# slowli/elastic-elgamal

Measured on AMD Instinct MI355X. Metric: EncryptedChoice ballot verifications/sec, higher is better.
Workload: dtype u32; 1 GPU; 1000000 single-choice 5-option EncryptedChoice ballots per GPU per step, resident in HBM (BASELINE.json configs[1]); verify + homomorphic tally + tally all-gather; ballots_per_gpu=1000000, total_ballots=1000000, options=5, ballot_bytes=736, seed=20260612, tampered=0, parallelism=single

## Files before the change

### elastic_elgamal_amd/csrc/eg_hip.hip

```cpp
#include <hip/hip_runtime.h>

#include <algorithm>
#include <atomic>
#include <chrono>
#include <cstdio>
#include <cstdlib>
#include <cstring>
#include <functional>
#include <memory>
#include <mutex>
#include <string>
#include <thread>
#include <condition_variable>
#include <deque>
#include <list>
#include <unordered_map>
#include <vector>

#include "../../include/eg_hip.h"
#include "host_plan.hpp"
#include "wire_json.hpp"
#include "kernels.cuh"
#include "pippenger.cuh"

// ... 146 lines not shown
  return EG_OK;
}

static void comb_table_free(uint4* tab) { if (tab) (void)hipFree(tab - COMB_HEADER_QUADS); }
static int comb_table_build(const u32* d_base_words, int bits, hipStream_t s, uint4** out, bool soft_nomem = false) {
  *out = nullptr;
  if (bits < 8 || bits > 26) return fail(EG_ERR_BAD_ARG, "comb width out of range");
  const int windows = comb_windows(bits), entries = comb_entries(bits);
  const size_t lanes = (size_t)windows * (entries / COMB_RUN);
  uint4* base = nullptr;
  u32 *d_bases = nullptr, *scratch = nullptr;
  hipError_t he = hipMalloc((void**)&base, ((size_t)windows * entries * 8 + COMB_HEADER_QUADS) * sizeof(uint4));
  if (he == hipSuccess) he = hipMalloc((void**)&d_bases, (size_t)windows * PT_WORDS * sizeof(u32));
  if (he == hipSuccess) he = hipMalloc((void**)&scratch, (size_t)COMB_RUN * EG_NL * lanes * sizeof(u32));
  if (he != hipSuccess) {
    if (base) (void)hipFree(base);
    if (d_bases) (void)hipFree(d_bases);
    if (scratch) (void)hipFree(scratch);
    if (he == hipErrorOutOfMemory && soft_nomem) { (void)hipGetLastError(); return EG_ERR_NOMEM; }
    HIPCHK(he);
  }
  hipLaunchKernelGGL(k_comb_window_bases, dim3(1), dim3(64), 0, s, d_base_words, bits, d_bases);
  hipLaunchKernelGGL(k_build_fixed_table, dim3((unsigned)((lanes + NT - 1) / NT)), dim3(NT), 0, s, d_bases, bits, base + COMB_HEADER_QUADS, scratch);
  const hipError_t se = hipStreamSynchronize(s);
  (void)hipFree(d_bases); (void)hipFree(scratch);
  if (se != hipSuccess) { (void)hipFree(base); HIPCHK(se); }
  *out = base + COMB_HEADER_QUADS;
  return EG_OK;
}

using eghost::StageDev; using eghost::LevelDev;
using eghost::FAM_TABLE1; using eghost::FAM_TABLEN; using eghost::FAM_DIRECT1; using eghost::FAM_GENERIC; using eghost::FAM_ENCODE; using eghost::N_FAM;
using eghost::EG_MULTI_GROUP; using eghost::job_family;

struct Engine {
  eg_ctx* ctx = nullptr;
  eghost::Plan plan;
  int n_options = 0;
  egplan::WireItem *d_pt_items = nullptr, *d_sc_items = nullptr;
  egplan::DeriveClass* d_dclasses = nullptr;
  egplan::DeriveTerm* d_dterms = nullptr;
  egplan::JobClass* d_jobs = nullptr;
  egplan::VarTerm* d_vterms = nullptr;
  egplan::HashInst* d_insts = nullptr;
  egplan::HashOp* d_ops = nullptr;
  egplan::StatusRule* d_rules = nullptr;
  u32* d_tally_slots = nullptr;
  unsigned short* d_base_slots = nullptr;
  egplan::SumBase* d_sum_bases = nullptr;
  unsigned short* d_sum_members = nullptr;
  egplan::SumBase* d_acc_sums = nullptr;
  unsigned short* d_acc_members = nullptr;
  int n_sums = 0;
  unsigned short* d_defer_slots = nullptr;
  int max_defer = 0;
  unsigned char* d_blob = nullptr;
  uint4 *d_tabK = nullptr, *d_cpts = nullptr;
  uint4* d_tabK_big = nullptr;
  bool use_big = false;
  size_t items_seen = 0;
  u32* d_prefixes = nullptr;
  u32* d_key_words = nullptr;
  std::vector<StageDev> stages;
  std::vector<LevelDev> levels;
  int prefix_inst_first = 0, prefix_inst_count = 0;
  struct WorkSet {
    uint4 *pts = nullptr, *cmp = nullptr, *chal = nullptr;
    u32 *states = nullptr, *flags = nullptr, *bad_item = nullptr;
    uint4 *btab = nullptr, *dpt = nullptr, *sacc = nullptr;
    u32* encw = nullptr;
    u32* partial = nullptr;
    u32* tally = nullptr;
    hipStream_t stream = nullptr;
    hipEvent_t done = nullptr;
  } set[2];
  int n_sets = 2;
  Knobs knobs;
  uint8_t key_bytes[32] = {0};
  int teeth = 6;
  hipEvent_t fork = nullptr;
  u32 cap = 0, max_cap = 0;
// ... 13 lines not shown
  bool reserved = false;
  hipEvent_t last_done = nullptr, saved_ev = nullptr;
  bool last_used = false;
  hipStream_t copy_stream = nullptr;
  unsigned char* d_wire = nullptr;
  u32* d_status = nullptr;
  size_t staging_ballots = 0;
  u32* gen_ws = nullptr;
  size_t gen_ws_bytes = 0;
  u32* d_gen_desc = nullptr;
};

static int grid_for(size_t lanes, int cap_blocks);
static int gen_workspace(Engine* e, size_t n, unsigned words, int* blocks_out) {
  const size_t budget = (size_t)2 << 30;
  int blocks = grid_for(n, e->ctx->cus * 4);
  const size_t per_block = (size_t)NT * words * sizeof(u32);
  if ((size_t)blocks * per_block > budget) blocks = (int)std::max<size_t>(1, budget / per_block);
  const size_t need = (size_t)blocks * per_block;
  if (need > e->gen_ws_bytes) {
    HIPCHK(hipDeviceSynchronize());
    if (e->gen_ws) (void)hipFree(e->gen_ws);
    e->gen_ws = nullptr; e->gen_ws_bytes = 0;
    HIPCHK(hipMalloc((void**)&e->gen_ws, need));
    e->gen_ws_bytes = need;
  }
  *blocks_out = blocks;
  return EG_OK;
}

static void engine_free(Engine* e) {
  if (!e) return;
  void* ptrs[] = {e->d_pt_items, e->d_sc_items, e->d_dclasses, e->d_dterms, e->d_jobs, e->d_vterms, e->d_insts, e->d_ops,
                  e->d_rules, e->d_tally_slots, e->d_base_slots, e->d_sum_bases, e->d_sum_members, e->d_acc_sums, e->d_acc_members, e->d_defer_slots, e->d_blob, e->d_cpts, e->d_prefixes, e->d_key_words,
                  e->tally_saved, e->tally_saved2, e->tally_saved3, e->d_tally_enc, e->d_wire, e->d_status, e->gen_ws, e->d_gen_desc};
  for (void* p : ptrs) if (p) (void)hipFree(p);
  for (auto& w : e->set) {
    void* sp[] = {w.pts, w.cmp, w.chal, w.states, w.flags, w.bad_item, w.btab, w.dpt, w.sacc, w.encw, w.partial, w.tally};
    for (void* p : sp) if (p) (void)hipFree(p);
    if (w.stream) (void)hipStreamDestroy(w.stream);
    if (w.done) (void)hipEventDestroy(w.done);
  }
  if (e->fork) (void)hipEventDestroy(e->fork);
  if (e->last_done) (void)hipEventDestroy(e->last_done);
  if (e->saved_ev) (void)hipEventDestroy(e->saved_ev);
  comb_table_free(e->d_tabK); comb_table_free(e->d_tabK_big);
  if (e->copy_stream) (void)hipStreamDestroy(e->copy_stream);
  if (e->json_ring) (void)hipHostFree(e->json_ring);
  if (e->json_status_ring) (void)hipHostFree(e->json_status_ring);
  for (hipStream_t st : e->json_ctl) if (st) (void)hipStreamDestroy(st);
  delete e;
}

static EngineBufs make_bufs(const Engine* e, int set, const void* d_ballots, u32 n, void* d_status) {
  const Engine::WorkSet& w = e->set[set];
  EngineBufs B;
  B.wire = reinterpret_cast<const u32*>(d_ballots);
  B.stride_words = (u32)(e->plan.stride / 4);
  B.n = n;
  B.cap = e->cap;
  B.pts = w.pts; B.cmp = w.cmp; B.chal = w.chal; B.states = w.states; B.flags = w.flags; B.bad_item = w.bad_item;
  B.status = reinterpret_cast<u32*>(d_status);
  B.tabG = e->use_big ? e->ctx->tabG_big : e->ctx->tabG; B.tabK = e->use_big ? e->d_tabK_big : e->d_tabK; B.cpts = e->d_cpts; B.prefixes = e->d_prefixes; B.blob = e->d_blob;
  B.ws = e->ctx->ws + (size_t)set * (e->ctx->msm_blocks / e->n_sets) * WS_QUADS * NT;
  B.btab = w.btab;
  B.sacc = w.sacc;
  B.dpt = w.dpt;
// ... 40 lines not shown
                     (void**)&w.btab, (void**)&w.dpt, (void**)&w.encw, (void**)&w.sacc};
    for (size_t i = 0; i < sizeof(sizes) / sizeof(sizes[0]); ++i) {
      const hipError_t he = hipMalloc(bufs[i], sizes[i]);
      if (he == hipErrorOutOfMemory) {
        (void)hipGetLastError();
        engine_release_sets(e);
        return fail(EG_ERR_NOMEM, "device memory exhausted while reserving the chunk workspace");
      }
      HIPCHK(he);
    }
  }
  e->cap = (u32)cap;
  return EG_OK;
}

static unsigned blocks_of(size_t n) { return (unsigned)std::max<size_t>(1, (n + NT - 1) / NT); }
static int grid_for(size_t lanes, int cap_blocks) {
  size_t blocks = (lanes + NT - 1) / NT;
  if (blocks < 1) blocks = 1;
  if ((size_t)cap_blocks < blocks) blocks = (size_t)cap_blocks;
  return (int)blocks;
}

static int engine_create(eg_ctx* ctx, eghost::Plan&& plan, const uint8_t pk[32], int n_options, Engine** out) {
  std::unique_ptr<Engine, void (*)(Engine*)> e(new Engine(), engine_free);
  e->ctx = ctx;
  e->plan = std::move(plan);
  e->n_options = n_options;
  eghost::Plan& P = e->plan;
  hipStream_t s = ctx->stream;
  HIPCHK(hipSetDevice(ctx->device));
  if (P.pk_off >= 0) memcpy(P.blob.data() + P.pk_off, pk, 32);

  const eghost::FlatPlan F = eghost::flatten_plan(P);
  {
    const std::string why = eghost::check_flat_plan(P, F);
    if (!why.empty()) return fail(EG_ERR_BAD_ARG, "internal: inconsistent verification plan: " + why);
  }
  e->stages = F.stages;
  e->levels = F.levels;
  e->max_defer = F.max_defer;
  e->prefix_inst_first = F.prefix_inst_first;
  e->prefix_inst_count = F.prefix_inst_count;
  const std::vector<egplan::JobClass>& jobs = F.jobs;
  const std::vector<egplan::HashInst>& insts = F.insts;
  const std::vector<egplan::HashOp>& ops = F.ops;
  const std::vector<uint16_t>& defer_slots = F.defer_slots;
  const std::vector<egplan::DeriveClass>& dclasses = F.dclasses;
  int rc;
  if ((rc = upload(&e->d_pt_items, P.pt_items, s))) return rc;
  if ((rc = upload(&e->d_sc_items, P.sc_items, s))) return rc;
  if ((rc = upload(&e->d_dclasses, dclasses, s))) return rc;
  if ((rc = upload(&e->d_dterms, P.dterms, s))) return rc;
  if ((rc = upload(&e->d_jobs, jobs, s))) return rc;
  if ((rc = upload(&e->d_vterms, P.vterms, s))) return rc;
  if ((rc = upload(&e->d_insts, insts, s))) return rc;
  if ((rc = upload(&e->d_ops, ops, s))) return rc;
  if ((rc = upload(&e->d_rules, P.rules, s))) return rc;
  if ((rc = upload(&e->d_tally_slots, P.tally_slots, s))) return rc;
  if ((rc = upload(&e->d_base_slots, F.build_slots, s))) return rc;
  if ((rc = upload(&e->d_sum_bases, F.sums, s))) return rc;
  if ((rc = upload(&e->d_sum_members, F.sum_members, s))) return rc;
  if ((rc = upload(&e->d_acc_sums, F.acc_sums, s))) return rc;
  if ((rc = upload(&e->d_acc_members, F.acc_members, s))) return rc;
  e->n_sums = (int)F.sums.size();
  if ((rc = upload(&e->d_defer_slots, defer_slots, s))) return rc;
  if ((rc = upload(&e->d_blob, P.blob, s))) return rc;

  u32* d_pk = nullptr;
  u32* d_flags = nullptr;
  HIPCHK(hipMalloc((void**)&d_pk, 32));
  HIPCHK(hipMalloc((void**)&d_flags, 8));
  HIPCHK(hipMalloc((void**)&e->d_key_words, 2 * PT_WORDS * sizeof(u32)));
  HIPCHK(hipMemcpyAsync(d_pk, pk, 32, hipMemcpyHostToDevice, s));
  hipLaunchKernelGGL(k_setup_points, dim3(1), dim3(64), 0, s, d_pk, e->d_key_words, d_flags);
  u32 hflags[2] = {0, 0};
  HIPCHK(hipMemcpyAsync(hflags, d_flags, 8, hipMemcpyDeviceToHost, s));
  HIPCHK(hipStreamSynchronize(s));
  (void)hipFree(d_pk); (void)hipFree(d_flags);
  if (!hflags[0]) return fail(EG_ERR_BAD_PUBLIC_KEY, "public key is not a valid ristretto255 encoding");
  if (hflags[1]) return fail(EG_ERR_BAD_PUBLIC_KEY, "public key is the identity");
  if ((rc = comb_table_build(e->d_key_words + PT_WORDS, EG_COMB_BITS, s, &e->d_tabK))) return rc;

  {
    u64* d_m = nullptr;
    std::vector<uint64_t> mults = P.const_mults;
    if (mults.empty()) mults.push_back(0);
    HIPCHK(hipMalloc((void**)&d_m, mults.size() * 8));
    HIPCHK(hipMemcpyAsync(d_m, mults.data(), mults.size() * 8, hipMemcpyHostToDevice, s));
    HIPCHK(hipMalloc((void**)&e->d_cpts, mults.size() * PT_QUADS * sizeof(uint4)));
    hipLaunchKernelGGL(k_const_points, dim3((unsigned)((mults.size() + NT - 1) / NT)), dim3(NT), 0, s, d_m, (int)mults.size(),
                       ctx->tabG, e->d_cpts);
    HIPCHK(hipStreamSynchronize(s));
// ... 133 lines not shown
    for (int k = 0; k < 2; ++k) {
      HIPCHK(hipStreamWaitEvent(e->set[k].stream, e->fork, 0));
      TRY_(ws_acquire(ctx, 1u << k, e->set[k].stream));
    }
  } else if (n) {
    TRY_(ws_acquire(ctx, 3u, s));
    whole_ws = true;
  }
  const bool inject_failure = two && EG_FAULT_POINT(after_fork);
  const int msm_blocks = ctx->msm_blocks / (two ? 2 : 1);
  size_t chunk = 0;
  for (size_t off = 0; off < n; off += even, ++chunk) {
    const int set = two ? (int)(chunk & 1) : 0;
    hipStream_t cs = two ? e->set[set].stream : s;
    const Engine::WorkSet& w = e->set[set];
    const u32 cn = (u32)std::min<size_t>(even, n - off);
    EngineBufs B = make_bufs(e, set, reinterpret_cast<const unsigned char*>(d_ballots) + off * P.stride, cn,
                             reinterpret_cast<u32*>(d_status) + off);
    if (!two) B.ws = ctx->ws;
    const int wide = ctx->cus * 32;
    HIPCHK(hipMemsetAsync(w.bad_item, 0xff, (size_t)cn * sizeof(u32), cs));
    hipLaunchKernelGGL(k_decode_points, dim3(grid_for((size_t)P.pt_items.size() * cn, wide)), dim3(NT), 0, cs, B, e->d_pt_items,
                       (int)P.pt_items.size());
    hipLaunchKernelGGL(k_check_scalars, dim3(grid_for((size_t)P.sc_items.size() * cn, wide)), dim3(NT), 0, cs, B, e->d_sc_items,
                       (int)P.sc_items.size());
    for (auto& lv : e->levels)
      if (lv.count)
        hipLaunchKernelGGL(k_derive_points, dim3(grid_for((size_t)lv.count * cn, wide)), dim3(NT), 0, cs, B, e->d_dclasses,
                           e->d_dterms, lv.first, lv.count);
    for (auto& st : e->stages) {
      if (st.build_count) {
        size_t pi = 0;
        if ((rc = prof_begin(ctx, cs, PROF_TABLES, &pi))) return rc;
        EG_WITH_TEETH(e->teeth, hipLaunchKernelGGL(k_base_tables<T>, dim3(grid_for((size_t)st.build_count * cn, msm_blocks)), dim3(NT), 0, cs, B,
                                                   e->d_base_slots + st.build_first, st.build_count));
        if ((rc = prof_end(ctx, cs, pi))) return rc;
      }
      if (st.sums_direct)
        EG_WITH_TEETH(e->teeth, hipLaunchKernelGGL(k_sum_tables<T>, dim3(grid_for((size_t)e->n_sums * cn, msm_blocks)), dim3(NT), 0, cs, B,
                                                   e->d_sum_bases, e->d_sum_members, e->n_sums));
      if (st.acc_count)
        EG_WITH_TEETH(e->teeth, hipLaunchKernelGGL(k_sum_accumulate<T>, dim3(grid_for((size_t)st.acc_count * T * cn, msm_blocks)), dim3(NT), 0, cs, B,
                                                   e->d_acc_sums + st.acc_first, e->d_acc_members, st.acc_count));
      if (st.sum_finish)
        EG_WITH_TEETH(e->teeth, hipLaunchKernelGGL(k_sum_finish<T>, dim3(grid_for((size_t)e->n_sums * cn, msm_blocks)), dim3(NT), 0, cs, B,
                                                   e->d_sum_bases, e->n_sums));
      if (st.fam_count[FAM_TABLE1]) {
        size_t pi = 0;
        if ((rc = prof_begin(ctx, cs, PROF_MSM, &pi))) return rc;
        EG_WITH_TEETH(e->teeth, hipLaunchKernelGGL((k_eq_table<false, T>), dim3(grid_for((size_t)st.fam_count[FAM_TABLE1] * cn, msm_blocks)), dim3(NT), 0, cs,
                                                   B, e->d_jobs, e->d_vterms, st.fam_first[FAM_TABLE1], st.fam_count[FAM_TABLE1], 1));
        if ((rc = prof_end(ctx, cs, pi))) return rc;
      }
      if (st.fam_count[FAM_TABLEN]) {
        const int group = std::min(st.max_terms, EG_MULTI_GROUP);
        EG_WITH_TEETH(e->teeth, hipLaunchKernelGGL((k_eq_table<true, T>), dim3(grid_for((size_t)st.fam_count[FAM_TABLEN] * cn, msm_blocks)), dim3(NT),
                                                   (size_t)group * 9 * NT * sizeof(u32), cs, B, e->d_jobs, e->d_vterms, st.fam_first[FAM_TABLEN],
                                                   st.fam_count[FAM_TABLEN], group));
      }
      if (st.fam_count[FAM_DIRECT1])
        hipLaunchKernelGGL(k_eq_direct, dim3(grid_for((size_t)st.fam_count[FAM_DIRECT1] * cn, msm_blocks)), dim3(NT), 0, cs, B,
                           e->d_jobs, e->d_vterms, st.fam_first[FAM_DIRECT1], st.fam_count[FAM_DIRECT1]);
      if (st.fam_count[FAM_GENERIC])
        EG_WITH_TEETH(e->teeth, hipLaunchKernelGGL(k_eq_generic<T>, dim3(grid_for((size_t)st.fam_count[FAM_GENERIC] * cn, msm_blocks)), dim3(NT), 0, cs, B,
                           e->d_jobs, e->d_vterms, st.fam_first[FAM_GENERIC], st.fam_count[FAM_GENERIC]));
      if (st.fam_count[FAM_ENCODE])
        hipLaunchKernelGGL(k_encode_plain, dim3(grid_for((size_t)st.fam_count[FAM_ENCODE] * cn, wide)), dim3(NT), 0, cs, B, e->d_jobs,
                           st.fam_first[FAM_ENCODE], st.fam_count[FAM_ENCODE]);
// ... 1169 lines not shown
    case 6: P = eghost::build_sumsq_plan(n_options, "test", &item); break;
    default: return fail(EG_ERR_BAD_ARG, "unknown plan kind");
  }
  size_t jobs = 0, insts = 0, var_terms = P.vterms.size(), table_terms = 0, derived = 0;
  size_t combs = 0, deferred = 0, plain_encodes = 0, inversion_groups = 0, derive_terms = P.dterms.size();
  size_t jobs_table1 = 0, chains = 0, chain_extra_terms = 0, loose_table_terms = 0, direct_terms = 0;
  std::string per_stage;
  for (auto& st : P.stages) {
    jobs += st.jobs.size(); insts += st.insts.size();
    per_stage += (per_stage.empty() ? "" : ",") + std::to_string(st.jobs.size());
    for (auto& j : st.jobs) {
      combs += (j.g.kind != egplan::SRC_NONE) + (j.k.kind != egplan::SRC_NONE);
      if (j.defer) ++deferred; else ++plain_encodes;
      switch (job_family(j, P.vterms)) {
        case FAM_TABLE1: ++jobs_table1; break;
        case FAM_TABLEN:
          for (int t0 = 0; t0 < (int)j.term_count; t0 += EG_MULTI_GROUP) {
            ++chains;
            chain_extra_terms += std::min<int>(EG_MULTI_GROUP, j.term_count - t0) - 1;
          }
          break;
        case FAM_DIRECT1: ++direct_terms; break;
        case FAM_GENERIC:
          for (unsigned t = 0; t < j.term_count; ++t)
            if (P.vterms[j.term_first + t].base == 0xffff) ++direct_terms; else ++loose_table_terms;
          break;
        default: break;
      }
    }
    inversion_groups += (st.deferred.size() + 31) / 32;
  }
  for (auto& t : P.vterms) table_terms += t.base != 0xffff;
  for (auto& l : P.derive_levels) derived += l.size();
  char tmp[2048];
  snprintf(tmp, sizeof tmp,
           "{\"stride\": %zu, \"wire_points\": %zu, \"wire_scalars\": %zu, \"derived_points\": %zu, \"derive_terms\": %zu, \"bases\": %zu, "
           "\"stages\": %zu, \"jobs\": %zu, \"jobs_per_stage\": [%s], \"var_terms\": %zu, \"table_terms\": %zu, "
           "\"combs\": %zu, \"deferred\": %zu, \"plain_encodes\": %zu, \"inversion_groups\": %zu, "
           "\"single_table_jobs\": %zu, \"chains\": %zu, \"chain_extra_terms\": %zu, \"loose_table_terms\": %zu, \"direct_terms\": %zu, "
           "\"sum_tables\": %zu, \"sum_table_members\": %zu, "
           "\"hash_programs\": %zu, \"prefixes\": %d, \"flags\": %d, \"rules\": %zu, \"tally_slots\": %zu, "
           "\"pt_slots\": %d, \"cmp_slots\": %d, \"chal_slots\": %d, \"state_slots\": %d, \"tables\": %zu, \"teeth\": %d, "
           "\"ring_group\": %d, \"table_groups\": %zu}",
           P.stride, P.pt_items.size(), P.sc_items.size(), derived, derive_terms, P.base_slots.size(), P.stages.size(), jobs, per_stage.c_str(),
           var_terms, table_terms, combs, deferred, plain_encodes, inversion_groups, jobs_table1, chains, chain_extra_terms,
           loose_table_terms, direct_terms, P.sum_bases.size(), P.sum_members.size(), insts, P.n_prefixes, P.n_flag_slots, P.rules.size(),
           P.tally_slots.size(), P.n_pt_slots, P.n_cmp_slots, P.n_chal_slots, P.n_state_slots, (size_t)P.n_tables(), eghost::plan_teeth(P),
           P.ring_group, P.group_stage.size());
  if (strlen(tmp) + 1 > cap) return fail(EG_ERR_BAD_ARG, "buffer too small");
  memcpy(buf, tmp, strlen(tmp) + 1);
  return EG_OK;
}

static int pack_json_common(const char* json, size_t json_len, int threads, size_t max_objects, size_t* n_objects,
                            std::vector<std::pair<size_t, size_t>>& spans) {
  if (!json_len) { if (n_objects) *n_objects = 0; return EG_OK; }
  if (!egwire::split_objects_parallel(json, json_len, threads, spans))
    return fail(EG_ERR_BAD_ARG, "the text is neither a JSON array of objects nor a sequence of JSON objects");
  if (n_objects) *n_objects = spans.size();
  if (spans.size() > max_objects) return fail(EG_ERR_BAD_ARG, "more objects in the text than max_objects (*n_objects says how many)");
  return EG_OK;
}
int eg_choice_pack_json(int n_options, int single, const char* json, size_t json_len, int threads, size_t max_objects,
                        uint8_t* packed, uint32_t* status, size_t* n_objects) {
  if (n_options < 1 || n_options > 4000 || (json_len && !json) || (max_objects && (!packed || !status)))
    return fail(EG_ERR_BAD_ARG, "bad argument");
  std::vector<std::pair<size_t, size_t>> spans;
  TRY(pack_json_common(json, json_len, threads, max_objects, n_objects, spans));
  const size_t stride = eghost::choice_ballot_size(n_options, single != 0);
  egwire::pack_parallel(json, spans, stride, threads, packed, status,
                        [&](egwire::Cursor& c, uint8_t* dst) { return egwire::pack_choice(c, n_options, single != 0, dst); });
  return EG_OK;
}
int eg_qv_pack_json(int n_options, uint64_t credits, const char* json, size_t json_len, int threads, size_t max_objects,
                    uint8_t* packed, uint32_t* status, size_t* n_objects) {
  if (n_options < 1 || n_options > 256 || credits < 1 || credits > 100000 || (json_len && !json) || (max_objects && (!packed || !status)))
    return fail(EG_ERR_BAD_ARG, "bad argument");
  std::vector<std::pair<size_t, size_t>> spans;
  TRY(pack_json_common(json, json_len, threads, max_objects, n_objects, spans));
  const eghost::QvShape sh = eghost::qv_shape(n_options, credits);
  const egwire::RangeShape vote{sh.vote_range.rings.size(), (size_t)sh.vote_range.rings_size()};
// ... 850 lines not shown
```

### elastic_elgamal_amd/csrc/host_plan.hpp

```cpp
#pragma once
#include <algorithm>
#include <cmath>
#include <cstdint>
#include <cstring>
#include <map>
#include <string>
#include <vector>
#include "plan.h"

namespace eghost {

using namespace egplan;

struct RingSpec { uint64_t size, step; };
struct RangeDecomposition {
  std::vector<RingSpec> rings;
  std::string to_string() const {
    std::string s;
    for (size_t i = 0; i < rings.size(); ++i) {
      if (rings[i].step > 1) s += std::to_string(rings[i].step) + " * ";
      s += "0.." + std::to_string(rings[i].size);
      if (i + 1 < rings.size()) s += " + ";
    }
    return s;
// ... 578 lines not shown
                               {OP_SAVE_PREFIX, 0, pre, 0}});
  const ScalarSrc c = wire_src(2, true), s = wire_src(3);
  const uint16_t xg = P.job(0, {}, s, c);
  const uint16_t xk = P.job(0, {P.term(dh, c), P.term(R, s)}, no_src(), no_src());
  const uint16_t flag = P.new_flag();
  P.stage(0).insts.push_back({{OP_LOAD_PREFIX, 0, pre, 0},
                              {OP_APPEND_WIRE, P.ref("K"), 0, 1},
                              {OP_APPEND_BLOB, P.ref("[r]G"), P.pk_ref(), 0},
                              {OP_APPEND_WIRE, P.ref("[r]K"), 1, 1},
                              {OP_APPEND_CMP, P.ref("[x]G"), xg, 0xffff},
                              {OP_APPEND_CMP, P.ref("[x]K"), xk, 0xffff},
                              {OP_CHALLENGE_CHECK, P.ref("c"), 2, flag}});
  P.rules.push_back({flag, 4});
  return P;
}

inline int plan_teeth(const Plan& P) {
  if (P.base_slots.empty()) return 6;
  return P.table_uses <= 2 * P.base_slots.size() + P.base_slots.size() / 2 ? 5 : 6;
}

enum { FAM_TABLE1 = 0, FAM_TABLEN = 1, FAM_DIRECT1 = 2, FAM_GENERIC = 3, FAM_ENCODE = 4, N_FAM = 5 };
constexpr int EG_MULTI_GROUP = 8;
inline int job_family(const JobClass& j, const std::vector<VarTerm>& vterms) {
  if (!j.defer) return FAM_ENCODE;
  if (j.term_count == 0) return FAM_GENERIC;
  for (unsigned t = 0; t < j.term_count; ++t)
    if (vterms[j.term_first + t].base == 0xffff) return j.term_count == 1 ? FAM_DIRECT1 : FAM_GENERIC;
  return j.term_count == 1 ? FAM_TABLE1 : FAM_TABLEN;
}
struct StageDev {
  int fam_first[N_FAM], fam_count[N_FAM], max_terms, inst_first, inst_count, defer_first, defer_count;
  int build_first, build_count, sums_direct, acc_first, acc_count, sum_finish;
};
struct LevelDev { int first, count; };
struct FlatPlan {
  std::vector<JobClass> jobs;
  std::vector<HashInst> insts;
  std::vector<HashOp> ops;
  std::vector<uint16_t> defer_slots;
  std::vector<DeriveClass> dclasses;
  std::vector<StageDev> stages;
  std::vector<LevelDev> levels;
  std::vector<uint16_t> build_slots;
  std::vector<SumBase> sums;
  std::vector<uint16_t> sum_members;
  std::vector<SumBase> acc_sums;
  std::vector<uint16_t> acc_members;
  int max_defer = 0, prefix_inst_first = 0, prefix_inst_count = 0;
};
inline FlatPlan flatten_plan(const Plan& P) {
  FlatPlan F;
  const size_t n_stages = std::max(P.stages.size(), (size_t)(P.sum_bases.empty() ? 0 : P.sum_stage + 1));
  std::vector<StageDev> tab(n_stages);
  for (auto& t : tab) t.build_first = t.build_count = t.sums_direct = t.acc_first = t.acc_count = t.sum_finish = 0;
  auto base_of = [&](uint16_t slot) -> int { auto it = P.base_index_of.find(slot); return it == P.base_index_of.end() ? -1 : (int)it->second; };
  for (size_t g = 0; g < P.group_stage.size(); ++g) {
    std::vector<uint16_t> slots(P.group_size((int)g));
    for (size_t i = 0; i < P.base_slots.size(); ++i)
      if (P.base_group[i] == g) slots[P.base_local[i]] = P.base_slots[i];
    if (slots.empty() || (size_t)P.group_stage[g] >= n_stages) continue;
    StageDev& t = tab[P.group_stage[g]];
    t.build_first = (int)F.build_slots.size(); t.build_count = (int)slots.size();
    F.build_slots.insert(F.build_slots.end(), slots.begin(), slots.end());
  }
  for (const SumBase& sb : P.sum_bases) {
    SumBase r = sb;
    r.first = (uint16_t)F.sum_members.size();
    for (unsigned t = 0; t < sb.count; ++t) {
      const int b = base_of(P.sum_members[sb.first + t]);
      F.sum_members.push_back(b < 0 ? (uint16_t)0xffff : P.base_local[b]);
    }
    F.sums.push_back(r);
  }
  if (!P.sum_bases.empty()) {
    if (!P.grouped()) tab[0].sums_direct = 1;
    else {
      std::vector<char> seen(P.sum_bases.size(), 0);
      for (size_t g = 0; g < P.group_stage.size(); ++g) {
        if ((size_t)P.group_stage[g] >= n_stages) continue;
        StageDev& t = tab[P.group_stage[g]];
        t.acc_first = (int)F.acc_sums.size();
        for (size_t k = 0; k < P.sum_bases.size(); ++k) {
          SumBase r;
          r.first = (uint16_t)F.acc_members.size(); r.count = 0; r.out_base = (uint16_t)k; r.pad = 0;
          for (unsigned m = 0; m < P.sum_bases[k].count; ++m) {
            const int b = base_of(P.sum_members[P.sum_bases[k].first + m]);
            if (b >= 0 && P.base_group[b] == g) { F.acc_members.push_back(P.base_local[b]); ++r.count; }
          }
          if (!r.count) continue;
          r.pad = seen[k] ? 0 : 1;
          seen[k] = 1;
          F.acc_sums.push_back(r);
        }
        t.acc_count = (int)F.acc_sums.size() - t.acc_first;
      }
      tab[P.sum_stage].sum_finish = 1;
    }
  }
  for (size_t si = 0; si < n_stages; ++si) {
    static const Stage empty_stage;
    const Stage& st = si < P.stages.size() ? P.stages[si] : empty_stage;
    StageDev sd = tab[si];
    sd.defer_first = (int)F.defer_slots.size(); sd.defer_count = (int)st.deferred.size();
    F.defer_slots.insert(F.defer_slots.end(), st.deferred.begin(), st.deferred.end());
    F.max_defer = std::max(F.max_defer, std::min(sd.defer_count, 32));
    sd.max_terms = 0;
    for (int f = 0; f < N_FAM; ++f) {
      sd.fam_first[f] = (int)F.jobs.size();
      for (auto& j : st.jobs)
        if (job_family(j, P.vterms) == f) {
          F.jobs.push_back(j);
          if (f == FAM_TABLEN) sd.max_terms = std::max<int>(sd.max_terms, j.term_count);
        }
      sd.fam_count[f] = (int)F.jobs.size() - sd.fam_first[f];
    }
    sd.inst_first = (int)F.insts.size(); sd.inst_count = (int)st.insts.size();
    for (auto& prog : st.insts) {
      F.insts.push_back({(uint32_t)F.ops.size(), (uint32_t)prog.size()});
      F.ops.insert(F.ops.end(), prog.begin(), prog.end());
    }
    F.stages.push_back(sd);
  }
  F.prefix_inst_first = (int)F.insts.size();
  F.prefix_inst_count = (int)P.prefix_programs.size();
  for (auto& prog : P.prefix_programs) {
    F.insts.push_back({(uint32_t)F.ops.size(), (uint32_t)prog.size()});
    F.ops.insert(F.ops.end(), prog.begin(), prog.end());
  }
  for (auto& lvl : P.derive_levels) {
    F.levels.push_back({(int)F.dclasses.size(), (int)lvl.size()});
    F.dclasses.insert(F.dclasses.end(), lvl.begin(), lvl.end());
  }
  return F;
}

inline std::string check_flat_plan(const Plan& P, const FlatPlan& F) {
  const size_t items = P.stride / 32;
  auto scalar_ok = [&](const ScalarSrc& s) {
    if (s.kind == SRC_NONE) return true;
    if (s.kind == SRC_WIRE) return (size_t)s.idx < items;
    return s.kind == SRC_CHAL && (int)s.idx < P.n_chal_slots;
  };
  if (P.stride % 32) return "stride is not a multiple of 32";
  for (auto& w : P.pt_items) if (w.item >= items || (int)w.slot >= P.n_pt_slots) return "wire point out of range";
  for (auto& w : P.sc_items) if (w.item >= items) return "wire scalar out of range";
  for (auto& d : F.dclasses) {
    if ((size_t)d.term_first + d.term_count > P.dterms.size() || (int)d.out_slot >= P.n_pt_slots) return "derive class out of range";
    for (unsigned t = 0; t < d.term_count; ++t) {
      const DeriveTerm& dt = P.dterms[d.term_first + t];
      if (dt.is_const ? dt.slot >= P.const_mults.size() : (int)dt.slot >= P.n_pt_slots) return "derive term out of range";
    }
  }
  for (uint16_t b : P.base_slots) if ((int)b >= P.n_pt_slots) return "base slot out of range";
  if (P.late_base) return "ordinary base registered after a sum base";
  if (P.base_group.size() != P.base_slots.size() || P.base_local.size() != P.base_slots.size()) return "base registry out of step";
  const size_t n_tab = P.n_tables();
  if (F.sums.size() != P.sum_bases.size()) return "sums lost in flattening";
  for (size_t i = 0; i < F.sums.size(); ++i) {
    const SumBase& sb = F.sums[i];
    if (sb.out_base != (P.grouped() ? i : P.base_slots.size() + i) || sb.out_base >= n_tab) return "sum base index out of order";
    if (sb.count == 0 || (size_t)sb.first + sb.count > F.sum_members.size()) return "sum base members out of range";
    for (unsigned t = 0; t < sb.count; ++t) {
      const uint16_t m = F.sum_members[sb.first + t];
      if (m == 0xffff) return "sum base member is not an ordinary base";
      if (!P.grouped() && m >= P.base_slots.size()) return "sum base member out of range";
    }
  }
  {
    size_t built = 0, acc_members = 0;
    std::vector<char> first_seen(F.sums.size(), 0);
    int last_acc_stage = -1, finish_stage = -1;
    for (size_t si = 0; si < F.stages.size(); ++si) {
      const StageDev& sd = F.stages[si];
      if (sd.build_count < 0 || (size_t)sd.build_first + sd.build_count > F.build_slots.size() || (size_t)sd.build_count > n_tab) return "table build range out of range";
      for (int k = 0; k < sd.build_count; ++k) if ((int)F.build_slots[sd.build_first + k] >= P.n_pt_slots) return "table build slot out of range";
      built += sd.build_count;
      if (sd.sums_direct && (P.grouped() || si != 0)) return "direct sum tables in a grouped plan";
      if (sd.acc_count < 0 || (size_t)sd.acc_first + sd.acc_count > F.acc_sums.size()) return "accumulate range out of range";
      for (int k = 0; k < sd.acc_count; ++k) {
        const SumBase& a = F.acc_sums[sd.acc_first + k];
        if (a.out_base >= F.sums.size() || a.count == 0 || (size_t)a.first + a.count > F.acc_members.size()) return "accumulate record out of range";
        for (unsigned m = 0; m < a.count; ++m) if ((int)F.acc_members[a.first + m] >= sd.build_count) return "accumulate member outside the group's tables";
        if ((a.pad != 0) != (first_seen[a.out_base] == 0)) return "accumulate first-mark out of order";
        first_seen[a.out_base] = 1;
        acc_members += a.count;
        last_acc_stage = (int)si;
      }
      if (sd.sum_finish) { if (finish_stage >= 0) return "sums finished twice"; finish_stage = (int)si; }
      if (sd.sum_finish && sd.build_count) return "sums finished in a stage that builds tables (they share the table slots)";
    }
    if (built != P.base_slots.size()) return "not every base table is built exactly once";
    if (P.grouped() && !F.sums.empty()) {
      size_t want = 0;
      for (auto& sb : F.sums) want += sb.count;
      if (acc_members != want || finish_stage <= last_acc_stage) return "sum accumulation incomplete or finished too early";
      for (char c : first_seen) if (!c) return "a sum has no members";
    } else if (finish_stage >= 0 || last_acc_stage >= 0) return "accumulators in an ungrouped plan";
  }
  size_t counted = 0, live = 0;
  enum { RES_ALL = -1, RES_SUMS = -2, RES_NONE = -3 };
  int resident = P.grouped() ? RES_NONE : RES_ALL;
  for (size_t si = 0; si < F.stages.size(); ++si) {
    const StageDev& sd = F.stages[si];
    if (sd.build_count) live = (size_t)sd.build_count + (sd.sums_direct ? F.sums.size() : 0);
    if (sd.sum_finish) live = F.sums.size();
    if (P.grouped()) {
      if (sd.build_count) {
        int g_here = -1;
        for (size_t g = 0; g < P.group_stage.size(); ++g)
          if (P.group_stage[g] == (int)si && P.group_size((int)g)) { if (g_here >= 0) return "two groups build their tables in one stage"; g_here = (int)g; }
        if (g_here < 0 || P.group_size(g_here) != (size_t)sd.build_count) return "a stage builds tables that are no group's";
        resident = g_here;
      }
      if (sd.sum_finish) resident = RES_SUMS;
    }
    for (int f = 0; f < N_FAM; ++f) {
      if (sd.fam_first[f] < 0 || (size_t)sd.fam_first[f] + sd.fam_count[f] > F.jobs.size()) return "family range out of range";
      counted += sd.fam_count[f];
      for (int k = 0; k < sd.fam_count[f]; ++k) {
        const JobClass& j = F.jobs[sd.fam_first[f] + k];
        if (job_family(j, P.vterms) != f) return "job in the wrong family";
        if ((size_t)j.term_first + j.term_count > P.vterms.size()) return "job terms out of range";
        if ((int)j.out_slot >= P.n_cmp_slots) return "job output out of range";
        if (!j.defer && (int)j.enc_slot >= P.n_pt_slots) return "encode job source out of range";
        if (!scalar_ok(j.g) || !scalar_ok(j.k)) return "job scalar out of range";
        for (unsigned t = 0; t < j.term_count; ++t) {
          const VarTerm& v = P.vterms[j.term_first + t];
          if (!scalar_ok(v.s) || v.s.kind == SRC_NONE) return "term scalar out of range";
          if (v.base == 0xffff ? (int)v.slot >= P.n_pt_slots : (v.base >= n_tab || v.base >= live)) return "term base out of range";
          if (v.base != 0xffff) {
            auto it = P.base_index_of.find(v.slot);
            if (it != P.base_index_of.end()) {
              const uint16_t i = it->second;
              if (P.base_local[i] != v.base) return "term names another base's table slot";
              if (P.grouped() && resident != (int)P.base_group[i]) return "term over a base whose group's tables are not resident at this stage";
            } else {
              const size_t first_sum = P.grouped() ? 0 : P.base_slots.size();
              if (v.base < first_sum || v.base - first_sum >= F.sums.size()) return "sum term names a table slot that is no sum's";
              if (P.grouped() && resident != RES_SUMS) return "sum term before the sums' tables are finished";
            }
          }
        }
      }
    }
    if ((size_t)sd.defer_first + sd.defer_count > F.defer_slots.size()) return "deferred range out of range";
    if ((size_t)sd.inst_first + sd.inst_count > F.insts.size()) return "program range out of range";
  }
  if (counted != F.jobs.size()) return "jobs lost in the family sort";
  for (uint16_t d : F.defer_slots) if ((int)d >= P.n_cmp_slots) return "deferred slot out of range";
  for (auto& in : F.insts) {
    if ((size_t)in.op_first + in.op_count > F.ops.size()) return "program ops out of range";
    for (uint32_t o = 0; o < in.op_count; ++o) {
      const HashOp& op = F.ops[in.op_first + o];
      auto blob_ok = [&](uint32_t ref) { return (size_t)(ref >> 12) + (ref & 0xfffu) <= P.blob.size(); };
// ... 24 lines not shown
```

### elastic_elgamal_amd/csrc/kernels.cuh

```cuda
#pragma once
#include <hip/hip_runtime.h>
#include "device_io.cuh"

#ifndef EG_EQ_WAVES
#define EG_EQ_WAVES 3
#endif
#ifndef EG_TAB_WAVES
#define EG_TAB_WAVES 2
#endif

namespace eg {

__device__ __forceinline__ void load_scalar(u32 s[8], const EngineBufs& B, u32 b, egplan::ScalarSrc src, bool halve = false) {
  if (src.kind == egplan::SRC_WIRE) load_wire_item(s, B, b, src.idx);
  else load32(s, B.chal, B.cap, src.idx, b);
  if (src.neg) { u32 t[8]; sc_neg(t, s);
#pragma unroll
    for (int i = 0; i < 8; ++i) s[i] = t[i]; }
  if (halve) { u32 t[8]; sc_halve(t, s);
#pragma unroll
    for (int i = 0; i < 8; ++i) s[i] = t[i]; }
}

__global__ void __launch_bounds__(NT, 2) k_decode_points(EngineBufs B, const egplan::WireItem* items, int n_items) {
// ... 90 lines not shown
      const BaseTable bt{B.btab + ((size_t)members[rec.first + t] * B.cap + b) * btab_quads<T>()};
      bt.load(e, g);
    });
  }
}
template <int T>
__global__ void __launch_bounds__(NT, EG_SUM_WAVES) k_sum_finish(EngineBufs B, const egplan::SumBase* sums, int n_sums) {
  const size_t total = (size_t)n_sums * B.n;
  WsRows tmp;
  tmp.init(B.ws);
  for (size_t j = (size_t)blockIdx.x * NT + threadIdx.x; j < total; j += (size_t)gridDim.x * NT) {
    const u32 k = (u32)(j / B.n), b = (u32)(j % B.n);
    BaseTable out{B.btab + ((size_t)sums[k].out_base * B.cap + b) * btab_quads<T>()};
    const BaseTable acc{B.sacc + ((size_t)k * B.cap + b) * (T * BTAB_ENTRY_QUADS)};
    ge_teeth_tables_sum<T>(out, tmp, 1, [&](int, int g, ge_cached& e) { acc.load(e, teeth_first_flip_index<T>(g)); });
  }
}

__device__ __forceinline__ void eq_fixed_terms(ge& acc, const EngineBufs& B, u32 b, const egplan::JobClass& jc) {
  const FixedTable tg(B.tabG), tk(B.tabK);
  if (jc.g.kind != egplan::SRC_NONE) {
    u32 s[8], dg[EG_COMB_WORDS];
    load_scalar(s, B, b, jc.g, true);
    sc_recode_comb(dg, s);
    ge_fixed_mul_add(acc, tg, dg);
  }
  if (jc.k.kind != egplan::SRC_NONE) {
    u32 s[8], dg[EG_COMB_WORDS];
    load_scalar(s, B, b, jc.k, true);
    sc_recode_comb(dg, s);
    ge_fixed_mul_add(acc, tk, dg);
  }
}

template <bool MULTI, int T>
__global__ void __launch_bounds__(NT, EG_EQ_WAVES) k_eq_table(EngineBufs B, const egplan::JobClass* classes, const egplan::VarTerm* terms,
                                                    int class_first, int n_classes, int group) {
  extern __shared__ u32 eq_signs[];
  const size_t total = (size_t)n_classes * B.n;
  for (size_t j = (size_t)blockIdx.x * NT + threadIdx.x; j < total; j += (size_t)gridDim.x * NT) {
    const u32 c = class_first + (u32)(j / B.n), b = (u32)(j % B.n);
    const egplan::JobClass jc = classes[c];
    ge acc;
    if (!MULTI) {
      const egplan::VarTerm vt = terms[jc.term_first];
      u32 s[8];
      load_scalar(s, B, b, vt.s, true);
      u64 rows[T];
      sc_recode_teeth<T>(rows, s);
      BaseTable bt{B.btab + ((size_t)vt.base * B.cap + b) * btab_quads<T>()};
      ge_teeth_mul<T>(acc, bt, rows);
    } else {
      const int nt = (int)jc.term_count;
#pragma unroll 1
      for (int t0 = 0; t0 < nt; t0 += group) {
        const int m = min(group, nt - t0);
#pragma unroll 1
        for (int t = 0; t < m; ++t) {
          u32 s[8], sg[9];
          load_scalar(s, B, b, terms[jc.term_first + t0 + t].s, true);
          sc_teeth_signs<T>(sg, s);
#pragma unroll
          for (int w = 0; w < 9; ++w) eq_signs[(t * 9 + w) * NT + threadIdx.x] = sg[w];
        }
        ge part;
        ge_teeth_mul_multi<T>(part, m,
            [&](int t, int col, int& idx, bool& neg) {
              sc_teeth_column<T>([&](int w) { return eq_signs[(t * 9 + w) * NT + threadIdx.x]; }, col, idx, neg);
            },
            [&](int t, int idx, ge_cached& e) {
              const BaseTable bt{B.btab + ((size_t)terms[jc.term_first + t0 + t].base * B.cap + b) * btab_quads<T>()};
              bt.load(e, idx);
            });
        if (t0 == 0) acc = part;
        else { ge sum; ge_add_full(sum, acc, part); acc = sum; }
      }
    }
    eq_fixed_terms(acc, B, b, jc);
    store_pt(B.dpt, B.cap, jc.out_slot, b, acc);
  }
}

__global__ void __launch_bounds__(NT, 2) k_eq_direct(EngineBufs B, const egplan::JobClass* classes, const egplan::VarTerm* terms,
                                                     int class_first, int n_classes) {
// ... 791 lines not shown
```

Before: 6.257 million ballots/s.

## Fuse single-use table-1 equation jobs into the per-ballot base table build kernel

When a stage builds per-ballot base tables, any TABLE1 equation job that is the sole user of a table is now evaluated in the same kernel lane that just built it. The lane does the teeth multiplication plus the fixed G/K terms and stores the result, and the job is dropped from the separate equation-kernel families. This is meant to cut a separate launch and let the lane use the just-written table while it is likely still cached, instead of re-reading it from HBM. The trade-offs are a larger table-build kernel, which may raise register pressure at its 2-wave launch bound, and extra plan bookkeeping and validation.

```diff
diff --git a/elastic_elgamal_amd/csrc/eg_hip.hip b/elastic_elgamal_amd/csrc/eg_hip.hip
--- a/elastic_elgamal_amd/csrc/eg_hip.hip
+++ b/elastic_elgamal_amd/csrc/eg_hip.hip
@@ -202,6 +202,11 @@
 using eghost::StageDev; using eghost::LevelDev;
 using eghost::FAM_TABLE1; using eghost::FAM_TABLEN; using eghost::FAM_DIRECT1; using eghost::FAM_GENERIC; using eghost::FAM_ENCODE; using eghost::N_FAM;
 using eghost::EG_MULTI_GROUP; using eghost::job_family;
+#ifdef EG_NO_TABLE_FUSION
+#define EG_TABLE_FUSION false
+#else
+#define EG_TABLE_FUSION true
+#endif
 
 struct Engine {
   eg_ctx* ctx = nullptr;
@@ -217,6 +222,7 @@
   egplan::StatusRule* d_rules = nullptr;
   u32* d_tally_slots = nullptr;
   unsigned short* d_base_slots = nullptr;
+  u32* d_fuse_jobs = nullptr;
   egplan::SumBase* d_sum_bases = nullptr;
   unsigned short* d_sum_members = nullptr;
   egplan::SumBase* d_acc_sums = nullptr;
@@ -296,7 +302,7 @@
 static void engine_free(Engine* e) {
   if (!e) return;
   void* ptrs[] = {e->d_pt_items, e->d_sc_items, e->d_dclasses, e->d_dterms, e->d_jobs, e->d_vterms, e->d_insts, e->d_ops,
-                  e->d_rules, e->d_tally_slots, e->d_base_slots, e->d_sum_bases, e->d_sum_members, e->d_acc_sums, e->d_acc_members, e->d_defer_slots, e->d_blob, e->d_cpts, e->d_prefixes, e->d_key_words,
+                  e->d_rules, e->d_tally_slots, e->d_base_slots, e->d_fuse_jobs, e->d_sum_bases, e->d_sum_members, e->d_acc_sums, e->d_acc_members, e->d_defer_slots, e->d_blob, e->d_cpts, e->d_prefixes, e->d_key_words,
                   e->tally_saved, e->tally_saved2, e->tally_saved3, e->d_tally_enc, e->d_wire, e->d_status, e->gen_ws, e->d_gen_desc};
   for (void* p : ptrs) if (p) (void)hipFree(p);
   for (auto& w : e->set) {
@@ -403,7 +409,7 @@
   HIPCHK(hipSetDevice(ctx->device));
   if (P.pk_off >= 0) memcpy(P.blob.data() + P.pk_off, pk, 32);
 
-  const eghost::FlatPlan F = eghost::flatten_plan(P);
+  const eghost::FlatPlan F = eghost::flatten_plan(P, EG_TABLE_FUSION);
   {
     const std::string why = eghost::check_flat_plan(P, F);
     if (!why.empty()) return fail(EG_ERR_BAD_ARG, "internal: inconsistent verification plan: " + why);
@@ -430,6 +436,7 @@
   if ((rc = upload(&e->d_rules, P.rules, s))) return rc;
   if ((rc = upload(&e->d_tally_slots, P.tally_slots, s))) return rc;
   if ((rc = upload(&e->d_base_slots, F.build_slots, s))) return rc;
+  if ((rc = upload(&e->d_fuse_jobs, F.fuse_jobs, s))) return rc;
   if ((rc = upload(&e->d_sum_bases, F.sums, s))) return rc;
   if ((rc = upload(&e->d_sum_members, F.sum_members, s))) return rc;
   if ((rc = upload(&e->d_acc_sums, F.acc_sums, s))) return rc;
@@ -629,8 +636,13 @@
       if (st.build_count) {
         size_t pi = 0;
         if ((rc = prof_begin(ctx, cs, PROF_TABLES, &pi))) return rc;
-        EG_WITH_TEETH(e->teeth, hipLaunchKernelGGL(k_base_tables<T>, dim3(grid_for((size_t)st.build_count * cn, msm_blocks)), dim3(NT), 0, cs, B,
-                                                   e->d_base_slots + st.build_first, st.build_count));
+        if (st.fused_count)
+          EG_WITH_TEETH(e->teeth, hipLaunchKernelGGL(k_base_tables_eq<T>, dim3(grid_for((size_t)st.build_count * cn, msm_blocks)), dim3(NT), 0, cs, B,
+                                                     e->d_base_slots + st.build_first, e->d_fuse_jobs + st.build_first, st.build_count,
+                                                     e->d_jobs, e->d_vterms));
+        else
+          EG_WITH_TEETH(e->teeth, hipLaunchKernelGGL(k_base_tables<T>, dim3(grid_for((size_t)st.build_count * cn, msm_blocks)), dim3(NT), 0, cs, B,
+                                                     e->d_base_slots + st.build_first, st.build_count));
         if ((rc = prof_end(ctx, cs, pi))) return rc;
       }
       if (st.sums_direct)
@@ -1866,6 +1878,8 @@
   }
   for (auto& t : P.vterms) table_terms += t.base != 0xffff;
   for (auto& l : P.derive_levels) derived += l.size();
+  size_t fused_jobs = 0;
+  for (auto& sd : eghost::flatten_plan(P, EG_TABLE_FUSION).stages) fused_jobs += sd.fused_count;
   char tmp[2048];
   snprintf(tmp, sizeof tmp,
            "{\"stride\": %zu, \"wire_points\": %zu, \"wire_scalars\": %zu, \"derived_points\": %zu, \"derive_terms\": %zu, \"bases\": %zu, "
@@ -1875,12 +1889,12 @@
            "\"sum_tables\": %zu, \"sum_table_members\": %zu, "
            "\"hash_programs\": %zu, \"prefixes\": %d, \"flags\": %d, \"rules\": %zu, \"tally_slots\": %zu, "
            "\"pt_slots\": %d, \"cmp_slots\": %d, \"chal_slots\": %d, \"state_slots\": %d, \"tables\": %zu, \"teeth\": %d, "
-           "\"ring_group\": %d, \"table_groups\": %zu}",
+           "\"ring_group\": %d, \"table_groups\": %zu, \"fused_jobs\": %zu}",
            P.stride, P.pt_items.size(), P.sc_items.size(), derived, derive_terms, P.base_slots.size(), P.stages.size(), jobs, per_stage.c_str(),
            var_terms, table_terms, combs, deferred, plain_encodes, inversion_groups, jobs_table1, chains, chain_extra_terms,
            loose_table_terms, direct_terms, P.sum_bases.size(), P.sum_members.size(), insts, P.n_prefixes, P.n_flag_slots, P.rules.size(),
            P.tally_slots.size(), P.n_pt_slots, P.n_cmp_slots, P.n_chal_slots, P.n_state_slots, (size_t)P.n_tables(), eghost::plan_teeth(P),
-           P.ring_group, P.group_stage.size());
+           P.ring_group, P.group_stage.size(), fused_jobs);
   if (strlen(tmp) + 1 > cap) return fail(EG_ERR_BAD_ARG, "buffer too small");
   memcpy(buf, tmp, strlen(tmp) + 1);
   return EG_OK;
diff --git a/elastic_elgamal_amd/csrc/host_plan.hpp b/elastic_elgamal_amd/csrc/host_plan.hpp
--- a/elastic_elgamal_amd/csrc/host_plan.hpp
+++ b/elastic_elgamal_amd/csrc/host_plan.hpp
@@ -634,6 +634,7 @@
 struct StageDev {
   int fam_first[N_FAM], fam_count[N_FAM], max_terms, inst_first, inst_count, defer_first, defer_count;
   int build_first, build_count, sums_direct, acc_first, acc_count, sum_finish;
+  int fused_first, fused_count;
 };
 struct LevelDev { int first, count; };
 struct FlatPlan {
@@ -645,17 +646,19 @@
   std::vector<StageDev> stages;
   std::vector<LevelDev> levels;
   std::vector<uint16_t> build_slots;
+  std::vector<uint32_t> fuse_jobs;
   std::vector<SumBase> sums;
   std::vector<uint16_t> sum_members;
   std::vector<SumBase> acc_sums;
   std::vector<uint16_t> acc_members;
   int max_defer = 0, prefix_inst_first = 0, prefix_inst_count = 0;
 };
-inline FlatPlan flatten_plan(const Plan& P) {
+constexpr uint32_t NO_FUSED_JOB = 0xffffffffu;
+inline FlatPlan flatten_plan(const Plan& P, bool fuse = true) {
   FlatPlan F;
   const size_t n_stages = std::max(P.stages.size(), (size_t)(P.sum_bases.empty() ? 0 : P.sum_stage + 1));
   std::vector<StageDev> tab(n_stages);
-  for (auto& t : tab) t.build_first = t.build_count = t.sums_direct = t.acc_first = t.acc_count = t.sum_finish = 0;
+  for (auto& t : tab) t.build_first = t.build_count = t.sums_direct = t.acc_first = t.acc_count = t.sum_finish = t.fused_first = t.fused_count = 0;
   auto base_of = [&](uint16_t slot) -> int { auto it = P.base_index_of.find(slot); return it == P.base_index_of.end() ? -1 : (int)it->second; };
   for (size_t g = 0; g < P.group_stage.size(); ++g) {
     std::vector<uint16_t> slots(P.group_size((int)g));
@@ -700,6 +703,7 @@
       tab[P.sum_stage].sum_finish = 1;
     }
   }
+  F.fuse_jobs.assign(F.build_slots.size(), NO_FUSED_JOB);
   for (size_t si = 0; si < n_stages; ++si) {
     static const Stage empty_stage;
     const Stage& st = si < P.stages.size() ? P.stages[si] : empty_stage;
@@ -708,10 +712,30 @@
     F.defer_slots.insert(F.defer_slots.end(), st.deferred.begin(), st.deferred.end());
     F.max_defer = std::max(F.max_defer, std::min(sd.defer_count, 32));
     sd.max_terms = 0;
+    std::vector<int> fused_slot(st.jobs.size(), -1);
+    if (fuse && sd.build_count) {
+      std::vector<int> uses(sd.build_count, 0), job_of(sd.build_count, -1);
+      for (size_t q = 0; q < st.jobs.size(); ++q) {
+        const JobClass& j = st.jobs[q];
+        if (job_family(j, P.vterms) != FAM_TABLE1) continue;
+        const VarTerm& v = P.vterms[j.term_first];
+        if ((int)v.base >= sd.build_count || F.build_slots[sd.build_first + v.base] != v.slot) continue;
+        if (uses[v.base]++ == 0) job_of[v.base] = (int)q;
+      }
+      for (int t = 0; t < sd.build_count; ++t)
+        if (uses[t] == 1) fused_slot[job_of[t]] = t;
+    }
+    sd.fused_first = (int)F.jobs.size();
+    for (size_t q = 0; q < st.jobs.size(); ++q)
+      if (fused_slot[q] >= 0) {
+        F.fuse_jobs[sd.build_first + fused_slot[q]] = (uint32_t)F.jobs.size();
+        F.jobs.push_back(st.jobs[q]);
+      }
+    sd.fused_count = (int)F.jobs.size() - sd.fused_first;
     for (int f = 0; f < N_FAM; ++f) {
       sd.fam_first[f] = (int)F.jobs.size();
-      for (auto& j : st.jobs)
-        if (job_family(j, P.vterms) == f) {
+      for (size_t q = 0; q < st.jobs.size(); ++q)
+        if (const JobClass& j = st.jobs[q]; fused_slot[q] < 0 && job_family(j, P.vterms) == f) {
           F.jobs.push_back(j);
           if (f == FAM_TABLEN) sd.max_terms = std::max<int>(sd.max_terms, j.term_count);
         }
@@ -757,6 +781,7 @@
   for (uint16_t b : P.base_slots) if ((int)b >= P.n_pt_slots) return "base slot out of range";
   if (P.late_base) return "ordinary base registered after a sum base";
   if (P.base_group.size() != P.base_slots.size() || P.base_local.size() != P.base_slots.size()) return "base registry out of step";
+  if (F.fuse_jobs.size() != F.build_slots.size()) return "fused job map out of step";
   const size_t n_tab = P.n_tables();
   if (F.sums.size() != P.sum_bases.size()) return "sums lost in flattening";
   for (size_t i = 0; i < F.sums.size(); ++i) {
@@ -817,12 +842,29 @@
       }
       if (sd.sum_finish) resident = RES_SUMS;
     }
-    for (int f = 0; f < N_FAM; ++f) {
-      if (sd.fam_first[f] < 0 || (size_t)sd.fam_first[f] + sd.fam_count[f] > F.jobs.size()) return "family range out of range";
-      counted += sd.fam_count[f];
-      for (int k = 0; k < sd.fam_count[f]; ++k) {
-        const JobClass& j = F.jobs[sd.fam_first[f] + k];
-        if (job_family(j, P.vterms) != f) return "job in the wrong family";
+    if (sd.fused_count < 0 || sd.fused_first < 0 || (size_t)sd.fused_first + sd.fused_count > F.jobs.size()) return "fused range out of range";
+    if (sd.fused_count && !sd.build_count) return "fused jobs in a stage that builds no tables";
+    {
+      int named = 0;
+      for (int k = 0; k < sd.build_count; ++k) {
+        const uint32_t q = F.fuse_jobs[sd.build_first + k];
+        if (q == NO_FUSED_JOB) continue;
+        ++named;
+        if (q < (uint32_t)sd.fused_first || q >= (uint32_t)(sd.fused_first + sd.fused_count)) return "fused job outside its stage's fused range";
+        const JobClass& j = F.jobs[q];
+        if ((size_t)j.term_first + j.term_count > P.vterms.size()) return "job terms out of range";
+        if (job_family(j, P.vterms) != FAM_TABLE1 || P.vterms[j.term_first].base != k || P.vterms[j.term_first].slot != F.build_slots[sd.build_first + k])
+          return "fused job does not read the table its lane builds";
+      }
+      if (named != sd.fused_count) return "fused jobs not named exactly once by the table lanes";
+    }
+    for (int f = 0; f <= N_FAM; ++f) {
+      const int first = f < N_FAM ? sd.fam_first[f] : sd.fused_first, count = f < N_FAM ? sd.fam_count[f] : sd.fused_count;
+      if (first < 0 || (size_t)first + count > F.jobs.size()) return "family range out of range";
+      counted += count;
+      for (int k = 0; k < count; ++k) {
+        const JobClass& j = F.jobs[first + k];
+        if (job_family(j, P.vterms) != (f < N_FAM ? f : (int)FAM_TABLE1)) return "job in the wrong family";
         if ((size_t)j.term_first + j.term_count > P.vterms.size()) return "job terms out of range";
         if ((int)j.out_slot >= P.n_cmp_slots) return "job output out of range";
         if (!j.defer && (int)j.enc_slot >= P.n_pt_slots) return "encode job source out of range";
diff --git a/elastic_elgamal_amd/csrc/kernels.cuh b/elastic_elgamal_amd/csrc/kernels.cuh
--- a/elastic_elgamal_amd/csrc/kernels.cuh
+++ b/elastic_elgamal_amd/csrc/kernels.cuh
@@ -146,6 +146,37 @@
     ge_fixed_mul_add(acc, tk, dg);
   }
 }
+template <int T>
+__device__ __forceinline__ void eq_table_term(ge& acc, const EngineBufs& B, u32 b, const egplan::VarTerm vt) {
+  u32 s[8];
+  load_scalar(s, B, b, vt.s, true);
+  u64 rows[T];
+  sc_recode_teeth<T>(rows, s);
+  BaseTable bt{B.btab + ((size_t)vt.base * B.cap + b) * btab_quads<T>()};
+  ge_teeth_mul<T>(acc, bt, rows);
+}
+
+template <int T>
+__global__ void __launch_bounds__(NT, EG_TAB_WAVES) k_base_tables_eq(EngineBufs B, const unsigned short* base_slots, const u32* fuse_jobs,
+                                                                      int n_bases, const egplan::JobClass* classes, const egplan::VarTerm* terms) {
+  const size_t total = (size_t)n_bases * B.n;
+  WsRows tmp;
+  tmp.init(B.ws);
+  for (size_t j = (size_t)blockIdx.x * NT + threadIdx.x; j < total; j += (size_t)gridDim.x * NT) {
+    const u32 k = (u32)(j / B.n), b = (u32)(j % B.n);
+    ge p;
+    load_pt(p, B.pts, B.cap, base_slots[k], b);
+    BaseTable bt{B.btab + ((size_t)k * B.cap + b) * btab_quads<T>()};
+    ge_teeth_tables_build<T>(bt, tmp, p);
+    const u32 c = fuse_jobs[k];
+    if (c == 0xffffffffu) continue;
+    const egplan::JobClass jc = classes[c];
+    ge acc;
+    eq_table_term<T>(acc, B, b, terms[jc.term_first]);
+    eq_fixed_terms(acc, B, b, jc);
+    store_pt(B.dpt, B.cap, jc.out_slot, b, acc);
+  }
+}
 
 template <bool MULTI, int T>
 __global__ void __launch_bounds__(NT, EG_EQ_WAVES) k_eq_table(EngineBufs B, const egplan::JobClass* classes, const egplan::VarTerm* terms,
@@ -157,13 +188,7 @@
     const egplan::JobClass jc = classes[c];
     ge acc;
     if (!MULTI) {
-      const egplan::VarTerm vt = terms[jc.term_first];
-      u32 s[8];
-      load_scalar(s, B, b, vt.s, true);
-      u64 rows[T];
-      sc_recode_teeth<T>(rows, s);
-      BaseTable bt{B.btab + ((size_t)vt.base * B.cap + b) * btab_quads<T>()};
-      ge_teeth_mul<T>(acc, bt, rows);
+      eq_table_term<T>(acc, B, b, terms[jc.term_first]);
     } else {
       const int nt = (int)jc.term_count;
 #pragma unroll 1
```

Result: no change. 6.296 million ballots/s, median of 6 (+0.6%).
